# Orange-OpenSource/AIVC

Measured on AMD Instinct MI355X. Metric: encode+decode fps @1080p YUV420 (RA GOP32), higher is better.
Workload: dtype f32; 1 GPU; 1920x1080 8-bit YUV420, coding structure 1_GOP_32: one 128-frame clip = 4 intra-period units of 33 frames (132 coded frames, the last 4 repeat the last frame) encoded + decoded per step; synthetic random-init stand-in for model ms_ssim-4 (widths {'n2': 64, 'n': 128, 'c_y': 64, 'c_short': 64, 'c_z': 32, 'n_h': 128}), last analysis conv calibrated so that 6 (MOFNet) / 12 (CodecNet) of the 64 y featu; parallelism=single GPU

## Files before the change

aivc_amd/csrc/gdn.hip:

```cpp
#include <stdlib.h>

#include "mfma_util.h"

namespace aivc {

struct GdnArgs {
  aivc_conv_params p;
  int M;
  int ntiles;
};

constexpr int GDN_BM = 64;

__device__ __forceinline__ int gdn_swz(int row) { return (row & 15) ^ ((row & 4) << 1); }

template <int C>
struct GdnCfg {
  static constexpr int NB = C / 32;
  static constexpr int PW = C == 64 ? 2 : 1;
  static constexpr int NW = NB * PW;
  static constexpr int TM = 2 / PW;
  static constexpr int ROWB = C * 4;
  static constexpr int STAGE = GDN_BM * ROWB;
  static constexpr int PIECES = STAGE / 1024;
  static constexpr int PPW = (PIECES + NW - 1) / NW;
  static constexpr int WGS = C == 192 ? 1 : 2;
};

template <int C, bool INV, bool RES>
__global__ __launch_bounds__(64 * GdnCfg<C>::NW, GdnCfg<C>::WGS) void gdn_resident_kernel(GdnArgs a) {
  using Cfg = GdnCfg<C>;
  constexpr int NB = Cfg::NB, PW = Cfg::PW, NW = Cfg::NW, TM = Cfg::TM, ROWB = Cfg::ROWB, STAGE = Cfg::STAGE, PIECES = Cfg::PIECES, PPW = Cfg::PPW;
  constexpr int NOCT = C / 8;
  extern __shared__ __attribute__((aligned(16))) char gsmem[];
  const uint32_t lds0 = (uint32_t)(uintptr_t)(__attribute__((address_space(3))) char *)gsmem;
  const aivc_conv_params &p = a.p;
  const int tid = threadIdx.x, lane = tid & 63;
  const int wave = __builtin_amdgcn_readfirstlane(tid >> 6);
  const int nb = wave % NB, pw = wave / NB;
  const int l31 = lane & 31, hh = lane >> 5;
  const int M = a.M;

  float4 gb[NOCT];
  {
    const float *g = p.w + (size_t)(32 * nb + l31) * C + 4 * hh;
#pragma unroll
    for (int o = 0; o < NOCT; ++o) gb[o] = *reinterpret_cast<const float4 *>(g + 8 * o);
  }
  const float cbeta = p.bias[32 * nb + l31];

  uint32_t d_voff[PPW];
#pragma unroll
  for (int k = 0; k < PPW; ++k) {
    const int q = wave + NW * k;
    const int b = q * 1024 + lane * 16;
    const int row = b / ROWB, chunk = ((b % ROWB) >> 4) ^ gdn_swz(row);
    d_voff[k] = (uint32_t)(row * ROWB + chunk * 16);
  }
  const uint32_t w_dst = __builtin_amdgcn_readfirstlane(lds0 + (uint32_t)wave * 1024u);
  auto issue = [&](int tile, int stage) {
    const int m0 = tile * GDN_BM;
    const float *src = p.x + (size_t)m0 * C;
    const uint32_t dst = w_dst + (uint32_t)(stage * STAGE);
    if (m0 + GDN_BM <= M) {
#pragma unroll
      for (int k = 0; k < PPW; ++k)
        if (PIECES % NW == 0 || wave + NW * k < PIECES) glds16(src, d_voff[k], dst + (uint32_t)(NW * k) * 1024u);
    } else {
      const int last = M - 1 - m0;
#pragma unroll
      for (int k = 0; k < PPW; ++k)
        if (PIECES % NW == 0 || wave + NW * k < PIECES)
          glds16(src, (uint32_t)min((int)(d_voff[k] / ROWB), last) * (uint32_t)ROWB + d_voff[k] % ROWB, dst + (uint32_t)(NW * k) * 1024u);
    }
  };

  const int frow = (PW == 2 ? 32 * pw : 0) + l31;
  int f_off[8];
#pragma unroll
  for (int o = 0; o < 8; ++o) f_off[o] = frow * ROWB + (((2 * o + hh) ^ gdn_swz(frow)) << 4);
  const int e_chunk = (8 * nb + (l31 >> 2)) ^ (hh ? 12 : 0);
  const int e_lane = 4 * hh * ROWB + (l31 & 3) * 4;
  const int rb0 = PW == 2 ? 32 * pw : 0;

  const int G = gridDim.x;
  int tile = blockIdx.x;
  if (tile >= a.ntiles) return;
  issue(tile, 0);
  int stage = 0;
  for (; tile < a.ntiles; tile += G, stage ^= 1) {
    asm volatile("s_waitcnt vmcnt(0)" ::: "memory");
    __builtin_amdgcn_s_barrier();
    if (tile + G < a.ntiles) issue(tile + G, stage ^ 1);
    const char *sb = gsmem + stage * STAGE;

    floatx16 acc[TM];
    typedef float f32x2 __attribute__((ext_vector_type(2)));
    struct Frag { f32x2 lo, hi; };
    Frag cur[TM], nxt[TM];
    auto read_frag = [&](Frag (&f)[TM], int o) {
#pragma unroll
      for (int i = 0; i < TM; ++i) {
        const float4 v = *reinterpret_cast<const float4 *>(sb + f_off[o & 7] + (o >> 3) * 256 + i * 32 * ROWB);
        f[i].lo = (f32x2){v.x, v.y};
        f[i].hi = (f32x2){v.z, v.w};
      }
    };
    read_frag(cur, 0);
#pragma unroll
    for (int o = 0; o < NOCT; ++o) {
      if (o + 1 < NOCT) read_frag(nxt, o + 1);
#pragma unroll
      for (int i = 0; i < TM; ++i) {
        cur[i].lo = cur[i].lo * cur[i].lo;
        cur[i].hi = cur[i].hi * cur[i].hi;
      }
      __builtin_amdgcn_sched_barrier(0);
#pragma unroll
      for (int s = 0; s < 4; ++s) {
        const float bv = s == 0 ? gb[o].x : (s == 1 ? gb[o].y : (s == 2 ? gb[o].z : gb[o].w));
#pragma unroll
        for (int i = 0; i < TM; ++i) {
          const float av = s == 0 ? cur[i].lo.x : (s == 1 ? cur[i].lo.y : (s == 2 ? cur[i].hi.x : cur[i].hi.y));
          if (o == 0 && s == 0) {
            const floatx16 zero = {0.0f, 0.0f, 0.0f, 0.0f, 0.0f, 0.0f, 0.0f, 0.0f, 0.0f, 0.0f, 0.0f, 0.0f, 0.0f, 0.0f, 0.0f, 0.0f};
            acc[i] = __builtin_amdgcn_mfma_f32_32x32x2f32(av, bv, zero, 0, 0, 0);
          } else {
            acc[i] = __builtin_amdgcn_mfma_f32_32x32x2f32(av, bv, acc[i], 0, 0, 0);
          }
        }
      }
      __builtin_amdgcn_sched_barrier(0);
#pragma unroll
      for (int i = 0; i < TM; ++i) cur[i] = nxt[i];
    }

    const int m0 = tile * GDN_BM;
    const int rows_left = M - m0;
    typedef __attribute__((address_space(1))) char gchar;
    typedef __attribute__((address_space(1))) float gfloat;
    typedef __attribute__((address_space(1))) const float cgfloat;
    gchar *yb = (gchar *)(uintptr_t)(p.y + (size_t)m0 * C);
    const gchar *rsb = (const gchar *)(uintptr_t)(p.res + (size_t)m0 * C);
    const uint32_t lane_b = (uint32_t)((4 * hh) * ROWB + (32 * nb + l31) * 4);
    auto epilogue = [&](auto WHOLE) {
      constexpr bool whole = decltype(WHOLE)::value;
      constexpr int EG = RES ? 4 : 8;
#pragma unroll
      for (int i = 0; i < TM; ++i)
#pragma unroll
      for (int r0 = 0; r0 < 16; r0 += EG) {
        const int rb = rb0 + 32 * i;
        float xv[EG], sv[EG], rv[EG];
        float mx = 1.0f, mn = 1.0f;
#pragma unroll
        for (int q = 0; q < EG; ++q) {
          const int r = r0 + q, rloc = (r & 3) + 8 * (r >> 2);
          const int cst = (r & 3) | (((r >> 2) & 1) << 3);
          xv[q] = *reinterpret_cast<const float *>(sb + (rb + rloc) * ROWB + e_lane + ((e_chunk ^ cst) << 4));
          if constexpr (RES) {
            const uint32_t off = lane_b + (uint32_t)((rb + rloc) * ROWB);
            rv[q] = (whole || rb + rloc + 4 * hh < rows_left) ? *reinterpret_cast<cgfloat *>(rsb + off) : 0.0f;
          }
        }
#pragma unroll
        for (int q = 0; q < EG; ++q) {
          sv[q] = acc[i][r0 + q] + cbeta;
          if constexpr (INV) gdn_range_pair(mx, mn, sv[q], sv[q]);
          else gdn_range(mx, mn, xv[q], sv[q]);
        }
        if (gdn_range_ok(mx, mn)) {
#pragma unroll
          for (int q = 0; q < EG; ++q) {
            const float nrm = sqrt_rn_safe(sv[q]);
            float v = INV ? xv[q] * nrm : div_rn_safe(xv[q], nrm);
            if constexpr (RES) v = v + rv[q];
            sv[q] = v;
          }
        } else {
#pragma unroll
          for (int q = 0; q < EG; ++q) {
            const float nrm = __builtin_sqrtf(sv[q]);
            float v = INV ? xv[q] * nrm : xv[q] / nrm;
            if constexpr (RES) v = v + rv[q];
            sv[q] = v;
            if (q & 1) __builtin_amdgcn_sched_barrier(0);
          }
        }
#pragma unroll
        for (int q = 0; q < EG; ++q) {
          const int r = r0 + q, rloc = (r & 3) + 8 * (r >> 2);
          const uint32_t off = lane_b + (uint32_t)((rb + rloc) * ROWB);
          if (whole || rb + rloc + 4 * hh < rows_left) *reinterpret_cast<gfloat *>(yb + off) = sv[q];
        }
        __builtin_amdgcn_sched_barrier(0);
      }
    };
    if (rows_left >= GDN_BM) epilogue(std::true_type{});
    else epilogue(std::false_type{});
  }
}

bool gdn_resident_supported(const aivc_conv_params &p) {
  if (p.mode != AIVC_MODE_GDN && p.mode != AIVC_MODE_IGDN) return false;
  if (p.c_in != 64 && p.c_in != 128) return false;
  if (p.c_out != p.c_in || !p.bias || p.mul || p.act1 != AIVC_ACT_NONE || p.act2 != AIVC_ACT_NONE) return false;
  if (((uintptr_t)p.x & 15u) || ((uintptr_t)p.w & 15u)) return false;
  const uint64_t pix = (uint64_t)p.n * p.h_in * p.w_in;
  return pix >= 1 && pix < 0x7FFFFFC0ull;
}

template <int C, bool INV, bool RES>
static int gdn_launch(const GdnArgs &a, hipStream_t s, int n_cu) {
  using Cfg = GdnCfg<C>;
  constexpr size_t lds = 2 * (size_t)Cfg::STAGE;
  static LdsOptIn opt_in;
  if (!opt_in.raise(reinterpret_cast<const void *>(gdn_resident_kernel<C, INV, RES>), lds)) return check_launch("gdn_resident lds attribute");
  unsigned grid = (unsigned)(n_cu * Cfg::WGS);
  if ((unsigned)a.ntiles < grid) grid = (unsigned)a.ntiles;
  hipLaunchKernelGGL((gdn_resident_kernel<C, INV, RES>), dim3(grid), dim3(64 * Cfg::NW), lds, s, a);
  return check_launch("gdn_resident");
}

int gdn_resident(const aivc_conv_params &p, hipStream_t s) {
  if (!gdn_resident_supported(p)) return AIVC_ERR_UNSUPPORTED;
  GdnArgs a;
  a.p = p;
  a.M = p.n * p.h_in * p.w_in;
  a.ntiles = (a.M + GDN_BM - 1) / GDN_BM;
  static std::atomic<int> n_cu{0};
  if (n_cu.load(std::memory_order_relaxed) == 0) {
    int dev = 0, cus = 0;
    n_cu = hipGetDevice(&dev) == hipSuccess && hipDeviceGetAttribute(&cus, hipDeviceAttributeMultiprocessorCount, dev) == hipSuccess && cus > 0 ? cus : 256;
  }
  const int cus = n_cu.load(std::memory_order_relaxed);
  const bool inv = p.mode == AIVC_MODE_IGDN, res = p.res != nullptr;
  auto go = [&](auto CC) {
    constexpr int C = decltype(CC)::value;
    if (inv) return res ? gdn_launch<C, true, true>(a, s, cus) : gdn_launch<C, true, false>(a, s, cus);
    return res ? gdn_launch<C, false, true>(a, s, cus) : gdn_launch<C, false, false>(a, s, cus);
  };
  if (p.c_in == 64) return go(std::integral_constant<int, 64>{});
  return go(std::integral_constant<int, 128>{});
}

}
```

Measured before the change: 104.5 frames/s.

## Overlap GDN output stores and residual loads with next tile's MFMA work

The GDN resident kernel now specializes the tile loop into whole tiles plus one optional tail tile. Whole tiles wait only until the previous tile's global stores drain (vmcnt of TILE_STORES) instead of waiting for all memory ops. Residual loads are moved ahead of the MFMA loop so their latency overlaps compute, and epilogue LDS addresses are precomputed. The cost is extra registers for the TM×16 residual values, and the counted wait relies on an exact count of outstanding stores, which risks ordering errors if that count is wrong.

```diff
diff --git a/aivc_amd/csrc/gdn.hip b/aivc_amd/csrc/gdn.hip
--- a/aivc_amd/csrc/gdn.hip
+++ b/aivc_amd/csrc/gdn.hip
@@ -25,6 +25,7 @@
   static constexpr int PIECES = STAGE / 1024;
   static constexpr int PPW = (PIECES + NW - 1) / NW;
   static constexpr int WGS = C == 192 ? 1 : 2;
+  static constexpr int TILE_STORES = 16 * TM;
 };
 
 template <int C, bool INV, bool RES>
@@ -87,12 +88,36 @@
   int tile = blockIdx.x;
   if (tile >= a.ntiles) return;
   issue(tile, 0);
-  int stage = 0;
-  for (; tile < a.ntiles; tile += G, stage ^= 1) {
-    asm volatile("s_waitcnt vmcnt(0)" ::: "memory");
+  __builtin_amdgcn_s_waitcnt(0x0F70);
+
+  auto do_tile = [&](int tile, int stage, auto WHOLE) {
+    constexpr bool whole = decltype(WHOLE)::value;
+    if constexpr (whole) asm volatile("s_waitcnt vmcnt(%0)" ::"n"(Cfg::TILE_STORES) : "memory");
+    else asm volatile("s_waitcnt vmcnt(0)" ::: "memory");
     __builtin_amdgcn_s_barrier();
     if (tile + G < a.ntiles) issue(tile + G, stage ^ 1);
     const char *sb = gsmem + stage * STAGE;
+
+    const int m0 = tile * GDN_BM;
+    const int rows_left = M - m0;
+    typedef __attribute__((address_space(1))) char gchar;
+    typedef __attribute__((address_space(1))) float gfloat;
+    typedef __attribute__((address_space(1))) const float cgfloat;
+    gchar *yb = (gchar *)(uintptr_t)(p.y + (size_t)m0 * C);
+    const gchar *rsb = (const gchar *)(uintptr_t)(p.res + (size_t)m0 * C);
+    const uint32_t lane_b = (uint32_t)((4 * hh) * ROWB + (32 * nb + l31) * 4);
+    auto rloc = [](int r) { return (r & 3) + 8 * (r >> 2); };
+
+    float rv[TM][16];
+    if constexpr (RES) {
+#pragma unroll
+      for (int i = 0; i < TM; ++i)
+#pragma unroll
+        for (int r = 0; r < 16; ++r) {
+          const int row = rb0 + 32 * i + rloc(r);
+          rv[i][r] = (whole || row + 4 * hh < rows_left) ? *reinterpret_cast<cgfloat *>(rsb + (size_t)(row * ROWB) + (size_t)lane_b) : 0.0f;
+        }
+    }
 
     floatx16 acc[TM];
     typedef float f32x2 __attribute__((ext_vector_type(2)));
@@ -135,70 +160,59 @@
       for (int i = 0; i < TM; ++i) cur[i] = nxt[i];
     }
 
-    const int m0 = tile * GDN_BM;
-    const int rows_left = M - m0;
-    typedef __attribute__((address_space(1))) char gchar;
-    typedef __attribute__((address_space(1))) float gfloat;
-    typedef __attribute__((address_space(1))) const float cgfloat;
-    gchar *yb = (gchar *)(uintptr_t)(p.y + (size_t)m0 * C);
-    const gchar *rsb = (const gchar *)(uintptr_t)(p.res + (size_t)m0 * C);
-    const uint32_t lane_b = (uint32_t)((4 * hh) * ROWB + (32 * nb + l31) * 4);
-    auto epilogue = [&](auto WHOLE) {
-      constexpr bool whole = decltype(WHOLE)::value;
-      constexpr int EG = RES ? 4 : 8;
-#pragma unroll
-      for (int i = 0; i < TM; ++i)
-#pragma unroll
-      for (int r0 = 0; r0 < 16; r0 += EG) {
-        const int rb = rb0 + 32 * i;
-        float xv[EG], sv[EG], rv[EG];
-        float mx = 1.0f, mn = 1.0f;
+    const char *xs[8];
+#pragma unroll
+    for (int j = 0; j < 8; ++j) xs[j] = sb + e_lane + ((e_chunk ^ ((j & 3) | ((j >> 2) << 3))) << 4);
+    constexpr int EG = RES ? 4 : 8;
+#pragma unroll
+    for (int i = 0; i < TM; ++i)
+#pragma unroll
+    for (int r0 = 0; r0 < 16; r0 += EG) {
+      const int rb = rb0 + 32 * i;
+      float xv[EG], sv[EG];
+      float mx = 1.0f, mn = 1.0f;
+#pragma unroll
+      for (int q = 0; q < EG; ++q) {
+        const int r = r0 + q;
+        xv[q] = *reinterpret_cast<const float *>(xs[(r & 3) + 4 * ((r >> 2) & 1)] + (rb + rloc(r)) * ROWB);
+      }
+#pragma unroll
+      for (int q = 0; q < EG; ++q) {
+        sv[q] = acc[i][r0 + q] + cbeta;
+        if constexpr (INV) gdn_range_pair(mx, mn, sv[q], sv[q]);
+        else gdn_range(mx, mn, xv[q], sv[q]);
+      }
+      if (gdn_range_ok(mx, mn)) {
 #pragma unroll
         for (int q = 0; q < EG; ++q) {
-          const int r = r0 + q, rloc = (r & 3) + 8 * (r >> 2);
-          const int cst = (r & 3) | (((r >> 2) & 1) << 3);
-          xv[q] = *reinterpret_cast<const float *>(sb + (rb + rloc) * ROWB + e_lane + ((e_chunk ^ cst) << 4));
-          if constexpr (RES) {
-            const uint32_t off = lane_b + (uint32_t)((rb + rloc) * ROWB);
-            rv[q] = (whole || rb + rloc + 4 * hh < rows_left) ? *reinterpret_cast<cgfloat *>(rsb + off) : 0.0f;
-          }
-        }
+          const float nrm = sqrt_rn_safe(sv[q]);
+          float v = INV ? xv[q] * nrm : div_rn_safe(xv[q], nrm);
+          if constexpr (RES) v = v + rv[i][r0 + q];
+          sv[q] = v;
+        }
+      } else {
 #pragma unroll
         for (int q = 0; q < EG; ++q) {
-          sv[q] = acc[i][r0 + q] + cbeta;
-          if constexpr (INV) gdn_range_pair(mx, mn, sv[q], sv[q]);
-          else gdn_range(mx, mn, xv[q], sv[q]);
-        }
-        if (gdn_range_ok(mx, mn)) {
-#pragma unroll
-          for (int q = 0; q < EG; ++q) {
-            const float nrm = sqrt_rn_safe(sv[q]);
-            float v = INV ? xv[q] * nrm : div_rn_safe(xv[q], nrm);
-            if constexpr (RES) v = v + rv[q];
-            sv[q] = v;
-          }
-        } else {
-#pragma unroll
-          for (int q = 0; q < EG; ++q) {
-            const float nrm = __builtin_sqrtf(sv[q]);
-            float v = INV ? xv[q] * nrm : xv[q] / nrm;
-            if constexpr (RES) v = v + rv[q];
-            sv[q] = v;
-            if (q & 1) __builtin_amdgcn_sched_barrier(0);
-          }
-        }
-#pragma unroll
-        for (int q = 0; q < EG; ++q) {
-          const int r = r0 + q, rloc = (r & 3) + 8 * (r >> 2);
-          const uint32_t off = lane_b + (uint32_t)((rb + rloc) * ROWB);
-          if (whole || rb + rloc + 4 * hh < rows_left) *reinterpret_cast<gfloat *>(yb + off) = sv[q];
-        }
-        __builtin_amdgcn_sched_barrier(0);
-      }
-    };
-    if (rows_left >= GDN_BM) epilogue(std::true_type{});
-    else epilogue(std::false_type{});
-  }
+          const float nrm = __builtin_sqrtf(sv[q]);
+          float v = INV ? xv[q] * nrm : xv[q] / nrm;
+          if constexpr (RES) v = v + rv[i][r0 + q];
+          sv[q] = v;
+          if (q & 1) __builtin_amdgcn_sched_barrier(0);
+        }
+      }
+#pragma unroll
+      for (int q = 0; q < EG; ++q) {
+        const int row = rb + rloc(r0 + q);
+        if (whole || row + 4 * hh < rows_left) *reinterpret_cast<gfloat *>(yb + (size_t)(row * ROWB) + (size_t)lane_b) = sv[q];
+      }
+      __builtin_amdgcn_sched_barrier(0);
+    }
+  };
+
+  const int nwhole = M / GDN_BM;
+  int stage = 0;
+  for (; tile < nwhole; tile += G, stage ^= 1) do_tile(tile, stage, std::true_type{});
+  if (tile < a.ntiles) do_tile(tile, stage, std::false_type{});
 }
 
 bool gdn_resident_supported(const aivc_conv_params &p) {
```

New measurement: 105.1 frames/s, median of 6. No clear change (+0.6%).
